# huj31415/nbody3d-webgpu

Hardware: AMD Instinct MI355X
Metric: pair-interactions/s (higher is better)
Workload: dtype f32; 1 GPU; N=262144 Plummer sphere, dt=1e-3, G=1, eps2=1e-4, i-sharded over 1 GPU(s); n=262144, kernel_variant=f32pk_symw_ipl16_j1_w2048_r32t128, parallelism=1gpu

## Files before the change

include/nbody3d_hip.h:

```cpp
#ifndef NBODY3D_HIP_H
#define NBODY3D_HIP_H

#include <stddef.h>
#include <stdint.h>

#ifdef __cplusplus
extern "C" {
#endif
#if defined(__GNUC__)
#pragma GCC visibility push(default)
#endif

#define NB_ABI_VERSION 2u
#define NB_ABI_MINOR 4u

typedef struct nb_sim nb_sim;

typedef enum nb_status {
    NB_OK = 0,
    NB_ERR_INVALID = 1,
    NB_ERR_NO_DEVICE = 2,
    NB_ERR_HIP = 3,
    NB_ERR_STATE = 4,
    NB_ERR_NOMEM = 5,
    NB_ERR_COMM = 6,
    NB_NOT_READY = 7
} nb_status;

typedef enum nb_precision { NB_F32 = 0, NB_F64 = 1 } nb_precision;

#define NB_FLAG_EXT_STREAM 1u
#define NB_FLAG_LDS_ONLY 4u
#define NB_FLAG_NO_FUSE 8u
#define NB_FLAG_POISON 16u

#define NB_FLAG_JPK_FENCED 32u

#define NB_FLAG_NO_SYM 64u

#define NB_FLAG_SYM_SHARD 128u

#define NB_FLAG_WHOLE_SWEEPS 256u

#define NB_FLAG_SINGLE_SWEEPS 512u

typedef enum nb_array { NB_BODIES = 0, NB_VEL = 1, NB_ACCEL = 2, NB_JERK = 3  } nb_array;

typedef enum nb_integrator { NB_INT_LEAPFROG = 0, NB_INT_HERMITE4 = 1 } nb_integrator;

typedef struct nb_config {
    uint32_t struct_size;
    uint32_t n;
    uint32_t precision;
    uint32_t tile;
    double eps2;
    int32_t device;
    uint32_t shard_begin;
    uint32_t shard_count;
    void *ext_stream;
    void *ext_bodies;
    uint32_t force_variant;
    uint32_t jsplit;
    uint32_t flags;
    uint32_t layer_budget_mib;
    uint32_t integrator;
    uint32_t reserved[3];
} nb_config;

uint32_t nb_abi_version(void);
uint32_t nb_abi_minor(void);

int nb_device_count(void);

int nb_create(const nb_config *cfg, nb_sim **out);

void nb_destroy(nb_sim *s);

// ... 128 lines not shown
```

nbody3d-webgpu_amd/csrc/kernels/symmetric.hip.h:

```cpp
#pragma once

namespace nb {

template <typename T> struct SymRowT { T x, y, z; };
using SymRow = SymRowT<float>;

constexpr uint32_t kFlushSteps = 4096;

template <int NG>
__device__ __forceinline__ void flush_resident_sums(float (*hi)[64], const int lane, const bool flushed, nb_f2 (&ax)[NG], nb_f2 (&ay)[NG], nb_f2 (&az)[NG])
{
    if (flushed) {
#pragma unroll
        for (int c = 0; c < NG; ++c) {
            hi[6 * c + 0][lane] += ax[c].x; hi[6 * c + 1][lane] += ay[c].x; hi[6 * c + 2][lane] += az[c].x;
            hi[6 * c + 3][lane] += ax[c].y; hi[6 * c + 4][lane] += ay[c].y; hi[6 * c + 5][lane] += az[c].y;
        }
    } else {
#pragma unroll
        for (int c = 0; c < NG; ++c) {
            hi[6 * c + 0][lane] = ax[c].x; hi[6 * c + 1][lane] = ay[c].x; hi[6 * c + 2][lane] = az[c].x;
            hi[6 * c + 3][lane] = ax[c].y; hi[6 * c + 4][lane] = ay[c].y; hi[6 * c + 5][lane] = az[c].y;
        }
    }
// ... 147 lines not shown
#pragma unroll
    for (int c = 0; c < NG; ++c) {
        out[(2 * c) * 64] = SymRow{ax[c].x, ay[c].x, az[c].x};
        out[(2 * c + 1) * 64] = SymRow{ax[c].y, ay[c].y, az[c].y};
    }
}

struct SymWK { uint32_t np, nsb, W, total_hi, total_lo, n_hi, zc, ups, r_layer0, t_layer0; };
#define SYMW_PLAN_PARAMS const uint32_t W_, const uint32_t ups_, const uint32_t nsb_, const uint32_t zc_, const uint32_t r_layer0_, const uint32_t t_layer0_
typedef uint32_t nb_u4 __attribute__((ext_vector_type(4)));
template <int TAIL>
__device__ __forceinline__ void symw_record_and_tail(const uint32_t* rec_at, nb_u4& rec, uint32_t (&tail)[TAIL])
{
    static_assert(TAIL == 1 || TAIL == 4, "f32: eps2; f64: G, eps2");
    constexpr int kTailOffset = 4 * 8 + 6 * 4;
    if constexpr (TAIL == 1) {
        asm volatile("s_load_dwordx4 %0, %2, 0x0\n\ts_load_dword %1, %3, %4\n\ts_waitcnt lgkmcnt(0)"
                     : "=&s"(rec), "=&s"(tail[0]) : "s"(rec_at), "s"(__builtin_amdgcn_kernarg_segment_ptr()), "n"(kTailOffset) : "memory");
    } else {
        nb_u4 t;
        asm volatile("s_load_dwordx4 %0, %2, 0x0\n\ts_load_dwordx4 %1, %3, %4\n\ts_waitcnt lgkmcnt(0)"
                     : "=&s"(rec), "=&s"(t) : "s"(rec_at), "s"(__builtin_amdgcn_kernarg_segment_ptr()), "n"(kTailOffset) : "memory");
        tail[0] = t.x; tail[1] = t.y; tail[2] = t.z; tail[3] = t.w;
    }
}

__device__ __forceinline__ SymWK symw_plan_words(uint32_t S, uint32_t cps, uint32_t W, uint32_t ups, uint32_t nsb, uint32_t zc, uint32_t r_layer0, uint32_t t_layer0)
{
    const uint32_t H = (nsb - 1u) >> 1, n_hi = (nsb & 1u) ? 0u : nsb >> 1;
    const uint32_t total_lo = (H + 1u) * cps + zc, total_hi = total_lo + (n_hi ? cps : 0u);
    return SymWK{(nsb + (zc ? 1u : 0u)) * S, nsb, W, total_hi, total_lo, n_hi, zc, ups, r_layer0, t_layer0};
}

template <int NG, int J, bool PAIR>
__device__ __forceinline__ void symw_sweeps(const uint32_t* __restrict__ gtab, const float4* __restrict__ bodies, SymRow* __restrict__ partial, SymRow* __restrict__ spill,
                                            SYMW_PLAN_PARAMS, uint32_t* __restrict__ queue, const uint32_t npieces, const uint32_t pieces_off)
{
    static_assert(!PAIR || J == 1, "paired sweeps: one traveler per lane and sweep");
    constexpr uint32_t S = 128u * NG;
    constexpr int GW = NG < 4 ? NG : 4;
    constexpr uint32_t CH = 64u * J;
    constexpr uint32_t CPS = S / CH;
    const SymWK pl = symw_plan_words(S, CPS, W_, ups_, nsb_, zc_, r_layer0_, t_layer0_);
    const int lane = threadIdx.x & 63, wi = threadIdx.x >> 6;
    const uint32_t w = __builtin_amdgcn_readfirstlane(blockIdx.x * 4u + wi);
    const bool active = w < pl.W;
    NB_STAMP(0);
    __shared__ float red[4][6 * NG][64];
    __shared__ uint32_t fin[4];
    const uint32_t ups = pl.ups, ush = (uint32_t)__builtin_ctz(ups), ustep = 64u >> ush,
                   tab1 = 2u * (pl.np / S);
    nb_u4 rec;
    uint32_t tail[1];
    symw_record_and_tail(gtab + tab1 + 4u * (active ? w : 0u), rec, tail);
    const float eps2 = __builtin_bit_cast(float, tail[0]);
    const nb_f2 e2 = nb_f2{eps2, eps2};
    const uint32_t first_lo = pl.n_hi * pl.total_hi, first_z = first_lo + (pl.nsb - pl.n_hi) * pl.total_lo;
    const uint32_t slot = rec.w;
    NB_STAMP_LIGHT(1);
    bool first_part = true;

    auto run = [&](uint32_t u, const uint32_t uend, const uint32_t piece_layer) -> uint32_t {
        uint32_t gfin = ~0u;
        while (u < uend) {
            const uint32_t p = u >> ush;
            uint32_t g, k, total;
            if (p < first_lo) { g = p / pl.total_hi; k = p - g * pl.total_hi; total = pl.total_hi; }
            else if (p < first_z) { const uint32_t r = p - first_lo; g = pl.n_hi + r / pl.total_lo; k = r - (g - pl.n_hi) * pl.total_lo; total = pl.total_lo; }
            else { g = pl.nsb; k = p - first_z; total = pl.zc; }
            const uint32_t ring = g < pl.nsb ? total - CPS - pl.zc : 0u;
            const uint32_t both_end = g < pl.nsb ? ring + pl.zc : 0u;
            uint32_t ug_end = (p - k + total) * ups;
            if (ug_end > uend) ug_end = uend;

            nb_f2 xi[NG], yi[NG], zi[NG], mi[NG], ax[NG], ay[NG], az[NG];
            {
                const float4* rb = bodies + (size_t)g * S + lane;
#pragma unroll
                for (int c = 0; c < NG; ++c) {
                    const float4 b0 = ld4(rb + (2 * c) * 64), b1 = ld4(rb + (2 * c + 1) * 64);
                    xi[c] = nb_f2{b0.x, b1.x}; yi[c] = nb_f2{b0.y, b1.y}; zi[c] = nb_f2{b0.z, b1.z}; mi[c] = nb_f2{b0.w, b1.w};
                    ax[c] = nb_f2{0, 0}; ay[c] = nb_f2{0, 0}; az[c] = nb_f2{0, 0};
                }
            }
            uint32_t since = 0;
            bool flushed = false;
            while (u < ug_end) {
                const uint32_t q0 = u & (ups - 1u);
                bool pair = false;
                if constexpr (PAIR) pair = q0 == 0u && ug_end - u >= 2u * ups && k + 1u < both_end;
                uint32_t nun = ups - q0;
                if (nun > ug_end - u) nun = ug_end - u;
                const uint32_t s0 = q0 * ustep, s1 = s0 + nun * ustep;
                u += pair ? 2u * ups : nun;
                if (since >= kFlushSteps) {
                    flush_resident_sums<NG>(red[wi], lane, flushed, ax, ay, az);
                    flushed = true;
                    since = 0;
                }
                since += pair ? 128u : s1 - s0;
                const bool sym = k < both_end, zsweep = k >= ring && sym;
                const uint32_t d = k / CPS;
                uint32_t tb = g + 1 + d;
                if (tb >= pl.nsb) tb -= pl.nsb;
                const uint32_t tstart = k < ring ? tb * S + (k % CPS) * CH : zsweep ? pl.nsb * S + (k - ring) * CH : g * S + (k - both_end) * CH;
                const uint32_t zrow = g * pl.zc + (k - ring);
                ++k;
                if constexpr (PAIR) {
                    if (pair) {
                        const bool zsweep1 = k >= ring;
                        const uint32_t d1 = k / CPS;
                        uint32_t tb1 = g + 1 + d1;
                        if (tb1 >= pl.nsb) tb1 -= pl.nsb;
                        const uint32_t tstart1 = zsweep1 ? pl.nsb * S + (k - ring) * CH : tb1 * S + (k % CPS) * CH;
                        const uint32_t zrow1 = g * pl.zc + (k - ring);
                        ++k;
                        const float4 t0 = ld4(bodies + tstart + lane), t1 = ld4(bodies + tstart1 + lane);
                        nb_f2 tx = nb_f2{t0.x, t1.x}, ty = nb_f2{t0.y, t1.y}, tz = nb_f2{t0.z, t1.z}, tm = nb_f2{t0.w, t1.w};
                        float bx0 = 0, bx1 = 0, by0 = 0, by1 = 0, bz0 = 0, bz1 = 0;
                        if (first_part) NB_STAMP(2);
                        for (uint32_t st = 0; st < 64u; ++st) {
                            nb_f2 sx = nb_f2{0, 0}, sy = nb_f2{0, 0}, sz = nb_f2{0, 0};
#pragma unroll
                            for (int c0g = 0; c0g < NG; c0g += GW) {
#pragma unroll
                                for (int f = 0; f < 2; ++f) {
                                    nb_f2 dx[GW], dy[GW], dz[GW], d2[GW], r[GW], si[GW], sj[GW];
#pragma unroll
                                    for (int c = 0; c < GW; ++c) dx[c] = symw_sub(f, tx, xi[c0g + c]);
#pragma unroll
                                    for (int c = 0; c < GW; ++c) dy[c] = symw_sub(f, ty, yi[c0g + c]);
#pragma unroll
                                    for (int c = 0; c < GW; ++c) dz[c] = symw_sub(f, tz, zi[c0g + c]);
#pragma unroll
                                    for (int c = 0; c < GW; ++c) d2[c] = __builtin_elementwise_fma(dx[c], dx[c], e2);
#pragma unroll
                                    for (int c = 0; c < GW; ++c) d2[c] = __builtin_elementwise_fma(dy[c], dy[c], d2[c]);
#pragma unroll
                                    for (int c = 0; c < GW; ++c) d2[c] = __builtin_elementwise_fma(dz[c], dz[c], d2[c]);
#pragma unroll
                                    for (int c = 0; c < GW; ++c) r[c] = d2[c] * d2[c];
#pragma unroll
                                    for (int c = 0; c < GW; ++c) r[c] = r[c] * d2[c];
#pragma unroll
                                    for (int c = 0; c < GW; ++c) r[c] = nb_f2{nb_rsq(r[c].x), nb_rsq(r[c].y)};
#pragma unroll
                                    for (int c = 0; c < GW; ++c) si[c] = symw_mul(f, tm, r[c]);
#pragma unroll
                                    for (int c = 0; c < GW; ++c) sj[c] = mi[c0g + c] * r[c];
#pragma unroll
                                    for (int c = 0; c < GW; ++c) ax[c0g + c] = __builtin_elementwise_fma(si[c], dx[c], ax[c0g + c]);
#pragma unroll
                                    for (int c = 0; c < GW; ++c) ay[c0g + c] = __builtin_elementwise_fma(si[c], dy[c], ay[c0g + c]);
#pragma unroll
                                    for (int c = 0; c < GW; ++c) az[c0g + c] = __builtin_elementwise_fma(si[c], dz[c], az[c0g + c]);
#pragma unroll
                                    for (int c = 0; c < GW; ++c) sx = symw_fnma(f, sj[c], dx[c], sx);
#pragma unroll
                                    for (int c = 0; c < GW; ++c) sy = symw_fnma(f, sj[c], dy[c], sy);
#pragma unroll
                                    for (int c = 0; c < GW; ++c) sz = symw_fnma(f, sj[c], dz[c], sz);
                                }
                            }
                            tx = nb_f2{wave_rot1(tx.x), wave_rot1(tx.y)}; ty = nb_f2{wave_rot1(ty.x), wave_rot1(ty.y)};
                            tz = nb_f2{wave_rot1(tz.x), wave_rot1(tz.y)}; tm = nb_f2{wave_rot1(tm.x), wave_rot1(tm.y)};
                            wave_rot1_add(bx0, sx.x); wave_rot1_add(bx1, sx.y); wave_rot1_add(by0, sy.x); wave_rot1_add(by1, sy.y);
                            wave_rot1_add(bz0, sz.x); wave_rot1_add(bz1, sz.y);
                            __builtin_amdgcn_sched_barrier(0);
                        }
                        if (first_part) { NB_STAMP_LIGHT(3); first_part = false; }
                        const uint32_t home = ((uint32_t)lane + 1u) & 63u;
                        SymRow* out0 = (zsweep ? spill + (size_t)zrow * CH : partial + (size_t)(pl.t_layer0 + d) * pl.np + tstart) + home;
                        SymRow* out1 = (zsweep1 ? spill + (size_t)zrow1 * CH : partial + (size_t)(pl.t_layer0 + d1) * pl.np + tstart1) + home;
                        *out0 = SymRow{bx0, by0, bz0};
                        *out1 = SymRow{bx1, by1, bz1};
                        continue;
                    }
                }
                float tx[J], ty[J], tz[J], tm[J];
                nb_f2 bx[J], by[J], bz[J];
                const uint32_t src = ((uint32_t)lane - s0) & 63u;
#pragma unroll
                for (int uu = 0; uu < J; ++uu) {
                    const float4 t = ld4(bodies + tstart + uu * 64 + src);
                    tx[uu] = t.x; ty[uu] = t.y; tz[uu] = t.z; tm[uu] = t.w;
                    bx[uu] = nb_f2{0, 0}; by[uu] = nb_f2{0, 0}; bz[uu] = nb_f2{0, 0};
                }
                auto steps = [&](auto both) {
                    constexpr bool BOTH = decltype(both)::value;
                    for (uint32_t st = s0; st < s1; ++st) {
#pragma unroll
                        for (int uu = 0; uu < J; ++uu) {
                            const nb_f2 px = nb_f2{tx[uu], tx[uu]}, py = nb_f2{ty[uu], ty[uu]}, pz = nb_f2{tz[uu], tz[uu]}, pm = nb_f2{tm[uu], tm[uu]};
#pragma unroll
                            for (int c0g = 0; c0g < NG; c0g += GW) {
                                nb_f2 dx[GW], dy[GW], dz[GW], d2[GW], r[GW], si[GW], sj[GW];
#pragma unroll
                                for (int c = 0; c < GW; ++c) dx[c] = px - xi[c0g + c];
#pragma unroll
                                for (int c = 0; c < GW; ++c) dy[c] = py - yi[c0g + c];
#pragma unroll
// ... 105 lines not shown
            members += same;
            mine += same && j < wi;
        }
        SymRow* out = partial + (size_t)(pl.r_layer0 + rec.z) * pl.np + (size_t)gfin * S + lane;
        for (int r = mine; r < 2 * NG; r += members) {
            float sx = 0.f, sy = 0.f, sz = 0.f;
#pragma unroll
            for (int j = 0; j < 4; ++j)
                if (fin[j] == gfin) { sx += red[j][3 * r + 0][lane]; sy += red[j][3 * r + 1][lane]; sz += red[j][3 * r + 2][lane]; }
            out[r * 64] = SymRow{sx, sy, sz};
        }
    }
    if (npieces) {
        for (;;) {
            uint32_t id = 0;
            if (lane == 0) id = __hip_atomic_fetch_add(queue, 1u, __ATOMIC_RELAXED, __HIP_MEMORY_SCOPE_AGENT);
            id = __builtin_amdgcn_readfirstlane(id);
            if (id >= npieces) break;
            const uint32_t pu = gtab[pieces_off + 2u * id], ll = gtab[pieces_off + 2u * id + 1u];
            (void)run(pu, pu + (ll >> 16), ll & 0xffffu);
        }
    }
    NB_STAMP(4);
}

#define SYMW_KERNEL_PARAMS const uint32_t* __restrict__ gtab, const float4* __restrict__ bodies, SymRow* __restrict__ partial, SymRow* __restrict__ spill, \
                           SYMW_PLAN_PARAMS, const float eps2_arg ,                       \
                           uint32_t* __restrict__ queue, const uint32_t npieces, const uint32_t pieces_off
#define SYMW_KERNEL_ARGS gtab, bodies, partial, spill, W_, ups_, nsb_, zc_, r_layer0_, t_layer0_, queue, npieces, pieces_off
template <int NG, int J>
__global__ __launch_bounds__(256) __attribute__((amdgpu_waves_per_eu(NG >= 4 ? 2 : 4, NG > 4 ? 2 : (NG < 4 ? 8 : 4))))
void nb_force_symw(SYMW_KERNEL_PARAMS)
{
    symw_sweeps<NG, J, false>(SYMW_KERNEL_ARGS);
}
template <int NG>
__global__ __launch_bounds__(256) __attribute__((amdgpu_waves_per_eu(2, NG > 4 ? 2 : 4)))
void nb_force_symw_pairs(SYMW_KERNEL_PARAMS)
{
    symw_sweeps<NG, 1, true>(SYMW_KERNEL_ARGS);
}

__device__ __forceinline__ double wave_rot1(double v)
{
    const long long b = __builtin_bit_cast(long long, v);
    const int lo = (int)(b & 0xffffffffll), hi = (int)(b >> 32);
    const unsigned rlo = (unsigned)__builtin_amdgcn_update_dpp(lo, lo, 0x13C, 0xF, 0xF, false);
    const unsigned rhi = (unsigned)__builtin_amdgcn_update_dpp(hi, hi, 0x13C, 0xF, 0xF, false);
    return __builtin_bit_cast(double, (long long)(((unsigned long long)rhi << 32) | rlo));
}

template <int IPL>
__global__ __launch_bounds__(256) __attribute__((amdgpu_waves_per_eu(2, 2)))
void nb_force_symw64(const uint32_t* __restrict__ gtab, const double4* __restrict__ bodies, SymRowT<double>* __restrict__ partial, SymRowT<double>* __restrict__ spill,
                     SYMW_PLAN_PARAMS, const double G_arg, const double eps2_arg ,
                     uint32_t* __restrict__ queue, const uint32_t npieces, const uint32_t pieces_off)
{
    constexpr uint32_t S = 64u * IPL, CH = 64u, CPS = S / CH;
    const SymWK pl = symw_plan_words(S, CPS, W_, ups_, nsb_, zc_, r_layer0_, t_layer0_);
    constexpr int GW = 4;
    const int lane = threadIdx.x & 63, wi = threadIdx.x >> 6;
    const uint32_t w = __builtin_amdgcn_readfirstlane(blockIdx.x * 4u + wi);
    const bool active = w < pl.W;
    __shared__ double red[4][3 * IPL][64];
    __shared__ uint32_t fin[4];
    const uint32_t ups = pl.ups, ush = (uint32_t)__builtin_ctz(ups), ustep = 64u >> ush,
                   tab1 = 2u * (pl.np / S);
    nb_u4 rec;
    uint32_t tail[4];
    symw_record_and_tail(gtab + tab1 + 4u * (active ? w : 0u), rec, tail);
    const double G = __builtin_bit_cast(double, (unsigned long long)tail[1] << 32 | tail[0]), eps2 = __builtin_bit_cast(double, (unsigned long long)tail[3] << 32 | tail[2]);
    const uint32_t first_lo = pl.n_hi * pl.total_hi, first_z = first_lo + (pl.nsb - pl.n_hi) * pl.total_lo;
    const uint32_t slot = rec.w;
// ... 586 lines not shown
```

nbody3d-webgpu_amd/csrc/nb_engine.hip:

```cpp
#include "nb_internal.h"
#include "nb_kernels.hip.h"
#include "../../include/nbody3d_hip_plan.h"

#include <hip/hip_ext.h>

#include <algorithm>
#include <cmath>
#include <cstdio>
#include <cstdlib>
#include <cstring>
#include <new>
#include <type_traits>

namespace {
thread_local std::string g_create_error = "";
}

namespace nbi {
int fail(nb_sim* s, int code, const std::string& msg)
{
    if (s) s->err = msg; else g_create_error = msg;
    return code;
}
void set_create_error(const std::string& msg) { g_create_error = msg; }
// ... 60 lines not shown
NB_PK_TABLE(pk_fused_kernel, nb_step_fused)

template <typename T>
const void* scalar_kernel(int ipl, int ls)
{
    if (ls == 1) {
        if (ipl == 1) return (const void*)&nb::nb_force<T, 1, 1>;
        if (ipl == 2) return (const void*)&nb::nb_force<T, 2, 1>;
        if (ipl == 4) return (const void*)&nb::nb_force<T, 4, 1>;
        return nullptr;
    }
    if (ipl != 1) return nullptr;
    if (ls == 4) return (const void*)&nb::nb_force<T, 1, 4>;
    if (ls == 16) return (const void*)&nb::nb_force<T, 1, 16>;
    if (ls == 64) return (const void*)&nb::nb_force<T, 1, 64>;
    return nullptr;
}

const void* sgpr_kernel(int ipl, int ws)
{
    if (ipl == 4 && ws == 5) return (const void*)&nb::nb_force_pk_sgpr<2, 4, true>;
    if (ipl == 4) return ws == 4 ? (const void*)&nb::nb_force_pk_sgpr<2, 4> : (const void*)&nb::nb_force_pk_sgpr<2, 1>;
    if (ipl == 8 && ws == 5) return (const void*)&nb::nb_force_pk_sgpr<4, 4, true>;
    if (ipl == 8) return ws == 4 ? (const void*)&nb::nb_force_pk_sgpr<4, 4> : (const void*)&nb::nb_force_pk_sgpr<4, 1>;
    return nullptr;
}

const void* rank_kernel_of(bool f64, int ipl)
{
    if (f64) return ipl == 8 ? (const void*)&nb::nb_force_symw64_rank<8> : nullptr;
    return ipl == 16 ? (const void*)&nb::nb_force_symw_rank<8> : ipl == 8 ? (const void*)&nb::nb_force_symw_rank<4> : nullptr;
}

const void* kernel_of(bool f64, const Shape& sh, bool single_sweeps = false)
{
    switch (sh.kind) {
        case kScalar: return f64 ? scalar_kernel<double>(sh.ipl, sh.ls) : scalar_kernel<float>(sh.ipl, sh.ls);
        case kPkLds: return f64 || (sh.ipl & 1) ? nullptr : pk_force_kernel(sh.ipl / 2, sh.ls, sh.x);
        case kFused: return f64 || (sh.ipl & 1) ? nullptr : pk_fused_kernel(sh.ipl / 2, sh.ls, sh.x);
        case kPkSgpr: return f64 || sh.ls != 1 || !(sh.x == 1 || sh.x == 4 || sh.x == 5) ? nullptr : sgpr_kernel(sh.ipl, sh.x);
        case kDirect:
            if (f64 || sh.ipl != 2 || sh.ls != 64) return nullptr;
            return sh.x == 1 ? (const void*)&nb::nb_step_direct<16> : sh.x == 2 ? (const void*)&nb::nb_step_direct<32> : nullptr;
        case kSym:
            if (sh.ls != 1) return nullptr;
            if (f64) return sh.ipl == 8 && sh.x == 3 ? (const void*)&nb::nb_force_symw64<8> : nullptr;
            if (sh.x == 4) return sh.ipl == 8 ? (const void*)&nb::nb_force_sym<4, 4, 2> : nullptr;
            if (sh.ipl == 4) return sh.x == 3 ? (const void*)&nb::nb_force_symw<2, 1> : nullptr;
            if (sh.ipl == 8 && sh.x == 3) return single_sweeps ? (const void*)&nb::nb_force_symw<4, 1> : (const void*)&nb::nb_force_symw_pairs<4>;
            if (sh.ipl == 16 && sh.x == 3) return single_sweeps ? (const void*)&nb::nb_force_symw<8, 1> : (const void*)&nb::nb_force_symw_pairs<8>;
            if (sh.ipl == 8) return sh.x == 1 ? (const void*)&nb::nb_force_symw<4, 2> : nullptr;
            if (sh.ipl == 16) return sh.x == 1 ? (const void*)&nb::nb_force_symw<8, 2> : nullptr;
            return nullptr;
        case kJpk:
            if (f64 || sh.ipl != 1 || sh.ls != 1) return nullptr;
            return sh.x == 4 ? (const void*)&nb::nb_step_jpk<4> : sh.x == 8 ? (const void*)&nb::nb_step_jpk<8>
                   : sh.x == 6 ? (const void*)&nb::nb_step_jpk<16> : nullptr;
        default: return nullptr;
    }
}

void plan_handle(nb_sim* s, const nb_config& cfg, int n_cu, double clock_hz, double device_mem)
{
    PlanInput in;
    if (device_mem > 0) in.device_mem = device_mem;
    in.n = s->n; in.sb = s->sb; in.sc = s->sc; in.f64 = s->f64; in.cfg = cfg; in.n_cu = n_cu; in.clock_hz = clock_hz;
    if (!s->no_device)
        in.occupancy = [f64 = s->f64](const Shape& sh, int block) {
            int occ = 0;
            const void* fn = kernel_of(f64, sh);
            if (!fn || hipOccupancyMaxActiveBlocksPerMultiprocessor(&occ, fn, block, 0) != hipSuccess) { (void)hipGetLastError(); return 0; }
            return occ;
        };
    LaunchPlan p = plan_launch(in);
    s->ipl = p.ipl; s->ls = p.ls; s->ws = p.ws; s->tl = p.tl;
    s->packed = p.packed; s->sgpr = p.sgpr; s->fused = p.fused; s->direct = p.direct; s->jpk = p.jpk; s->swap_acc = p.swap_acc;
    s->jsplit = p.jsplit; s->j_per_split = p.j_per_split; s->junits = p.junits; s->own_split0 = p.own_split0; s->own_splits = p.own_splits;
    s->sym = p.sym; s->symw = p.symw; s->sym_rank = p.sym_rank;
    s->sym_np = p.sym_np; s->sym_layers = p.sym_layers; s->sym_g0 = p.sym_g0; s->sym_g1 = p.sym_g1;
    static_assert(sizeof(s->sym_plan) == sizeof(p.sym_plan), "nb_sim::sym_plan mirrors LaunchPlan::sym_plan");
    memcpy(s->sym_plan, p.sym_plan, sizeof s->sym_plan);
    static_assert(sizeof(s->sym_rank_plan) == sizeof(p.sym_rank_plan), "nb_sim::sym_rank_plan mirrors LaunchPlan::sym_rank_plan");
    memcpy(s->sym_rank_plan, p.sym_rank_plan, sizeof s->sym_rank_plan);
// ... 62 lines not shown
        const void* b = jstream(s, s->cur);
        void* p = s->partial;
        const uint32_t* tab = s->sym_tab + ps.tab_off;
        uint32_t n = s->n, k_lo = ps.k_lo, k_hi = ps.k_hi, d0 = ps.d0;
        void* sp = s->sym_spill;
        if (s->f64) {
            double G = s->G, e2 = s->eps2;
            void* args[] = {&b, &p, &tab, &rp, &n, &G, &e2, &w0, &w1, &sp, &k_lo, &k_hi, &d0};
            launch_kernel(rank_kernel_of(true, sh.ipl), dim3(ceil_div(w1 - w0, 4u)), dim3(256), args, s->stream, t0, t1);
        } else {
            float e2 = (float)s->eps2;
            void* args[] = {&b, &p, &tab, &rp, &n, &e2, &w0, &w1, &sp, &k_lo, &k_hi, &d0};
            launch_kernel(rank_kernel_of(false, sh.ipl), dim3(ceil_div(w1 - w0, 4u)), dim3(256), args, s->stream, t0, t1);
        }
        return;
    }
    if (s->symw) {
        nb::SymWPlan pl;
        memcpy(&pl, s->sym_plan, sizeof pl);
        const void* b = jstream(s, s->cur);
        void* p = s->partial;
        const uint32_t* tab = s->sym_tab;
        void* sp = s->sym_spill;
        uint32_t* queue = s->sym_queue;
        uint32_t npieces = s->sym_pieces, pieces_off = 2u * (pl.np / ipb_of(sh)) + 4u * pl.W;
        if (npieces) (void)hipMemsetAsync(queue, 0, sizeof(uint32_t), s->stream);
        if (s->f64) {
            double G = s->G, e2 = s->eps2;
            void* args[] = {&tab, &b, &p, &sp, &pl.W, &pl.ups, &pl.nsb, &pl.zc, &pl.r_layer0, &pl.t_layer0, &G, &e2, &queue, &npieces, &pieces_off};
            launch_kernel(kernel_of(true, sh), dim3(ceil_div(pl.W, 4u)), dim3(256), args, s->stream, t0, t1);
        } else {
            float e2 = (float)s->eps2;
            void* args[] = {&tab, &b, &p, &sp, &pl.W, &pl.ups, &pl.nsb, &pl.zc, &pl.r_layer0, &pl.t_layer0, &e2, &queue, &npieces, &pieces_off};
            launch_kernel(kernel_of(false, sh, s->single_sweeps), dim3(ceil_div(pl.W, 4u)), dim3(256), args, s->stream, t0, t1);
        }
        return;
    }
    if (s->sym) {
        nb::SymPlan pl;
        memcpy(&pl, s->sym_plan, sizeof pl);
        const float4* b = (const float4*)jstream(s, s->cur);
        nb::SymRow* p = (nb::SymRow*)s->partial;
        float e2 = (float)s->eps2;
        uint32_t n = s->n;
        void* args[] = {&b, &p, &pl, &n, &e2};
        launch_kernel(kernel_of(false, sh), dim3(pl.nsb * pl.q), dim3(64 * sh.x), args, s->stream, t0, t1);
        return;
    }
    nb::SplitWindow win{0, 0xffffffffu, 0};
    uint32_t ny = s->jsplit;
    if (part == 1) { win.base = s->own_split0; ny = s->own_splits; }
    else if (part == 2) { win.hole_begin = s->own_split0; win.hole_count = s->own_splits; ny = s->jsplit - s->own_splits; }
    if (ny == 0) return;
    dim3 grid(ceil_div(s->sc, ipb_of(sh)), ny), block(nb::kBlock);
    const V4* b = (const V4*)jstream(s, s->cur);
    V4* p = (V4*)s->partial;
    T G = (T)s->G, e2 = (T)s->eps2;
    uint32_t n = s->n, sb = s->sb, sc = s->sc, jps = s->j_per_split;
    const V4* zr = (const V4*)s->zero_row;
    void* args[] = {&b, &p, &n, &sb, &sc, &G, &e2, &jps, &win, &zr};
    launch_kernel(kernel_of(s->f64, sh), grid, block, args, s->stream, t0, t1);
}

void ensure_pairs(nb_sim* s)
{
    if (!s->jpk || (s->pairs_ok && s->pairs_G == s->G)) return;
    const float4* b = (const float4*)s->bodies[s->cur];
// ... 520 lines not shown
        s->hermite = true;
        fj_shape(s->n, s->f64, n_cu, &s->fj_chunks, &s->fj_per);
        s->jsplit = s->fj_chunks; s->j_per_split = s->fj_per;
        s->variant = std::string("hermite4_") + (s->f64 ? "f64" : "f32pk") + "_c" + std::to_string(s->fj_chunks) + "_j" + std::to_string(s->fj_per);
        const size_t hrow = 4 * s->esz;
        NB_HIPC(hipMalloc(&s->bodies[0], hrow * s->n));
        s->own_bodies = true;
        for (void** p : {&s->vel, &s->acc, &s->jerk, &s->hx, &s->hv}) NB_HIPC(hipMalloc(p, hrow * s->n));
        NB_HIPC(hipMalloc(&s->fj_part, (size_t)2 * hrow * s->fj_chunks * s->n));
        NB_HIPC(hipMalloc(&s->zero_row, 64));
        NB_HIPC(hipMemsetAsync(s->zero_row, 0, 64, s->stream));
        s->diag_chunk = nb::kTile * std::min(16u, std::max(1u, s->n / 16384u));
        s->diag_blocks = ceil_div(s->sc, nb::kDiagRows) * ceil_div(s->n, s->diag_chunk);
        NB_HIPC(hipMalloc((void**)&s->diag, sizeof(double) * 5 * s->diag_blocks));
        *out = s;
        return NB_OK;
    }
    plan_handle(s, cfg, n_cu, clock_hz, (double)prop.totalGlobalMem);
    if (s->sym && (!s->sym_rank || s->sym_local) && !cfg.force_variant) {
        size_t free_b = 0, total_b = 0;
        auto need = [&]() { return 3.0 * s->esz * (double)sym_layer_rows(s) * s->sym_layers + 12.0 * s->esz * s->sym_np; };
        if (hipMemGetInfo(&free_b, &total_b) == hipSuccess && need() > 0.9 * (double)free_b) {
            nb_config fit = cfg;
            fit.layer_budget_mib = (uint32_t)std::max(1.0, 0.6 * (double)free_b / 1048576.0);
            plan_handle(s, fit, n_cu, clock_hz, (double)prop.totalGlobalMem);
            if (s->sym && need() > 0.9 * (double)free_b) {
                cfg.flags |= NB_FLAG_NO_SYM;
                plan_handle(s, cfg, n_cu, clock_hz, (double)prop.totalGlobalMem);
            }
        }
    }
    if (!kernel_of(s->f64, shape_of(s))) return bail(NB_ERR_INVALID, "nb_create: no kernel for shape " + s->variant);
    s->single_sweeps = (cfg.flags & NB_FLAG_SINGLE_SWEEPS) != 0;

    const size_t row = 4 * s->esz;
    if (cfg.ext_bodies) { s->bodies[0] = cfg.ext_bodies; s->own_bodies = false; }
    else {
        const size_t rows = s->sym ? s->sym_np : s->n;
        NB_HIPC(hipMalloc(&s->bodies[0], row * rows));
        if (s->sym) NB_HIPC(hipMemset(s->bodies[0], 0, row * rows));
        s->own_bodies = true;
        if (s->fused) NB_HIPC(hipMalloc(&s->bodies[1], row * s->n));
    }
    NB_HIPC(hipMalloc(&s->vel, row * s->sc));
    NB_HIPC(hipMalloc(&s->acc, row * s->sc));
    auto alloc_partial = [&](size_t bytes) -> hipError_t {
        if (s->partial) return hipErrorInvalidValue;
        s->partial_bytes = bytes;
        return hipMalloc(&s->partial, bytes);
    };
    if (s->sym) {
        NB_HIPC(alloc_partial((size_t)3 * s->esz * sym_layer_rows(s) * s->sym_layers));
        if (s->sym_rank) NB_HIPC(hipMalloc(&s->sym_A, 4 * s->esz * s->sym_np));
        if (s->sym_spill_rows) {
            NB_HIPC(hipMalloc(&s->sym_spill, (size_t)3 * s->esz * s->sym_spill_rows));
            NB_HIPC(hipMemset(s->sym_spill, 0, (size_t)3 * s->esz * s->sym_spill_rows));
        }
        if (s->symw && s->sym_pieces) {
            NB_HIPC(hipMalloc((void**)&s->sym_queue, 64));
            NB_HIPC(hipMemset(s->sym_queue, 0, 64));
        }
        if (s->symw) {
            NB_HIPC(hipMalloc((void**)&s->sym_tab, sizeof(uint32_t) * s->sym_tab_host.size()));
            NB_HIPC(hipMemcpy(s->sym_tab, s->sym_tab_host.data(), sizeof(uint32_t) * s->sym_tab_host.size(), hipMemcpyHostToDevice));
        }
    } else if (!s->fused) {
// ... 834 lines not shown
```

nbody3d-webgpu_amd/csrc/nb_internal.h:

```cpp
#pragma once
#include "../../include/nbody3d_hip.h"
#include "nb_plan.h"

#include <hip/hip_runtime.h>

#include <cstdint>
#include <string>
#include <vector>

struct nb_events { hipEvent_t e[8]; bool two, xchg, rs, blk; };

struct nb_rccl;

struct nb_frame_slot {
    float* h_bodies = nullptr;
    float* h_speed = nullptr;
    float* d_bodies = nullptr;
    float* d_speed = nullptr;
    hipEvent_t packed = nullptr;
    hipEvent_t landed = nullptr;
    uint64_t step = 0;
    bool in_flight = false, valid = false;
};

// ... 21 lines not shown
    uint32_t diag_blocks = 0, diag_chunk = 256;
    double dt = 0.0, G = 0.0;
    bool params_set = false, uploaded = false;
    uint64_t steps_done = 0;
    int ipl = 1, ls = 1;
    bool packed = false;
    bool sgpr = false;
    int ws = 1;
    int tl = 1;
    bool fused = false;
    bool direct = false;
    bool jpk = false;
    void* pairs[2] = {nullptr, nullptr};
    bool pairs_ok = false;
    double pairs_G = 0.0;
    void* jpartial = nullptr;
    uint32_t* tickets = nullptr;
    uint32_t junits = 0;
    bool poison = false;
    bool jpk_fenced = false;
    int acc_parity = 0;
    bool swap_acc = false;
    uint32_t jsplit = 1, j_per_split = 0;
    bool sym = false;
    uint32_t sym_np = 0, sym_layers = 0;
    uint32_t sym_plan[16] = {0};
    bool symw = false;
    uint32_t* sym_tab = nullptr;
    std::vector<uint32_t> sym_tab_host;
    void* sym_spill = nullptr;
    uint32_t sym_spill_rows = 0;
    uint32_t sym_pieces = 0;
    bool single_sweeps = false;
    uint32_t* sym_queue = nullptr;
    bool sym_rank = false;
    uint32_t sym_g0 = 0, sym_g1 = 0;
    uint32_t sym_rank_plan[16] = {0};
    std::vector<nbp::LaunchPlan::SymPass> sym_passes;
    uint32_t sym_pass = 0;
    bool sym_local = false;
    void* sym_A = nullptr;
    std::string variant, err;
    nb_exchange_fn xfn = nullptr;
    nb_exchange_wait_fn xwait = nullptr;
    void* xuser = nullptr;
    bool gather_pending = false;
    uint32_t own_split0 = 0, own_splits = 0;
    nb_rccl* rccl = nullptr;
    bool timing = false;
    struct graph_slot {
        hipGraph_t graph = nullptr;
        hipGraphExec_t exec = nullptr;
        double dt = 0.0, G = 0.0;
        int parity = 0;
    } graphs[2];
    bool graphs_ok = true;
    std::vector<nb_events> pool;
    std::vector<nb_events> pending;
    size_t pool_next = 0;
    hipStream_t frame_stream = nullptr;
    static constexpr int kFrameSlots = 4;
    nb_frame_slot frame[kFrameSlots];
    int frame_next = 0;
    int frame_latest = -1;
    int n_cu = 256;
    struct field_buf { void* p = nullptr; size_t cap = 0; } fld_pts, fld_acc, fld_phi, fld_part;
// ... 38 lines not shown
```

nbody3d-webgpu_amd/nbody3d_amd/capi.py:

```python
import ctypes as C
import os

import numpy as np

_PKG = os.path.dirname(os.path.abspath(__file__))
_LIB_PATH = os.environ.get("NB_ENGINE_LIB") or os.path.normpath(os.path.join(_PKG, "..", "csrc", "libnbody3d_hip.so"))

NB_F32, NB_F64 = 0, 1
NB_FLAG_EXT_STREAM = 1
NB_FLAG_LDS_ONLY = 4
NB_FLAG_NO_FUSE = 8
NB_FLAG_POISON = 16
NB_FLAG_JPK_FENCED = 32
NB_FLAG_NO_SYM = 64
NB_FLAG_SYM_SHARD = 128
NB_FLAG_WHOLE_SWEEPS = 256
NB_FLAG_SINGLE_SWEEPS = 512
NB_RCCL_ID_BYTES = 128
NB_RCCL_OVERLAP = 1
NB_MULTI_PEER, NB_MULTI_RCCL, NB_MULTI_PEER_OVERLAP = 0, 1, 2
NB_NOT_READY = 7
NB_FIELD_AT_BODIES, NB_FIELD_F64, NB_FIELD_DEVICE = 1, 2, 4
NB_INT_LEAPFROG, NB_INT_HERMITE4 = 0, 1
INTEGRATORS = {"leapfrog": NB_INT_LEAPFROG, "hermite4": NB_INT_HERMITE4}
STATUS = {0: "NB_OK", 1: "NB_ERR_INVALID", 2: "NB_ERR_NO_DEVICE", 3: "NB_ERR_HIP",
          4: "NB_ERR_STATE", 5: "NB_ERR_NOMEM", 6: "NB_ERR_COMM", 7: "NB_NOT_READY"}
ABI_VERSION = 2
ABI_MINOR = 3


class NBodyError(RuntimeError):
    def __init__(self, code, msg):
        super().__init__("%s: %s" % (STATUS.get(code, code), msg))
        self.code = code


class nb_config(C.Structure):
    _fields_ = [
        ("struct_size", C.c_uint32), ("n", C.c_uint32), ("precision", C.c_uint32), ("tile", C.c_uint32),
        ("eps2", C.c_double), ("device", C.c_int32), ("shard_begin", C.c_uint32), ("shard_count", C.c_uint32),
        ("ext_stream", C.c_void_p), ("ext_bodies", C.c_void_p),
        ("force_variant", C.c_uint32), ("jsplit", C.c_uint32), ("flags", C.c_uint32), ("layer_budget_mib", C.c_uint32),
        ("integrator", C.c_uint32), ("reserved", C.c_uint32 * 3),
    ]


class nb_plan_info(C.Structure):
    _fields_ = [("struct_size", C.c_uint32)] + [(k, C.c_uint32) for k in (
        "kind", "ipl", "ls", "x", "jsplit", "j_per_split", "own_split0", "own_splits",
        "sym", "symw", "sym_rank", "sym_np", "sym_layers", "sym_g0", "sym_g1")] + [
# ... 681 lines not shown
```

Baseline: 6811 billion pair-interactions/s.

## Rotate paired travelers through an LDS ring instead of DPP lane rotations

Result: no change. 6837 billion pair-interactions/s, median of 6 (+0.4%).

```diff
diff --git a/include/nbody3d_hip.h b/include/nbody3d_hip.h
--- a/include/nbody3d_hip.h
+++ b/include/nbody3d_hip.h
@@ -43,6 +43,8 @@
 #define NB_FLAG_WHOLE_SWEEPS 256u
 
 #define NB_FLAG_SINGLE_SWEEPS 512u
+
+#define NB_FLAG_DPP_PAIRS 1024u
 
 typedef enum nb_array { NB_BODIES = 0, NB_VEL = 1, NB_ACCEL = 2, NB_JERK = 3  } nb_array;
 
diff --git a/nbody3d-webgpu_amd/csrc/kernels/symmetric.hip.h b/nbody3d-webgpu_amd/csrc/kernels/symmetric.hip.h
--- a/nbody3d-webgpu_amd/csrc/kernels/symmetric.hip.h
+++ b/nbody3d-webgpu_amd/csrc/kernels/symmetric.hip.h
@@ -203,11 +203,77 @@
     return SymWK{(nsb + (zc ? 1u : 0u)) * S, nsb, W, total_hi, total_lo, n_hi, zc, ups, r_layer0, t_layer0};
 }
 
-template <int NG, int J, bool PAIR>
+enum SymwPairs { kNoPairs, kDppPairs, kLdsPairs };
+
+typedef float nb_f4 __attribute__((ext_vector_type(4)));
+template <int OFF>
+__device__ __forceinline__ void symw_ring_read(nb_f4& e0, nb_f4& e1, const uint32_t at)
+{
+    asm volatile("ds_read_b128 %0, %2 offset:%3\n\tds_read_b128 %1, %2 offset:%4" : "=&v"(e0), "=&v"(e1) : "v"(at), "n"(OFF), "n"(OFF + 2048) : "memory");
+}
+__device__ __forceinline__ void symw_ring_wait() { asm volatile("s_waitcnt lgkmcnt(0)" : : : "memory"); }
+template <int OFF>
+__device__ __forceinline__ void symw_ring_wait_step_read(uint32_t& at, nb_f4& n0, nb_f4& n1)
+{
+    asm volatile("s_waitcnt lgkmcnt(0)\n\tv_subrev_u32_e32 %0, 32, %0\n\tds_read_b128 %1, %0 offset:%3\n\tds_read_b128 %2, %0 offset:%4"
+                 : "+v"(at), "=&v"(n0), "=&v"(n1) : "n"(OFF), "n"(OFF + 2048) : "memory");
+}
+
+template <int NG>
+__device__ __forceinline__ void symw_pair_step(const nb_f2 tx, const nb_f2 ty, const nb_f2 tz, const nb_f2 tm, const nb_f2 e2,
+                                               const nb_f2 (&xi)[NG], const nb_f2 (&yi)[NG], const nb_f2 (&zi)[NG], const nb_f2 (&mi)[NG],
+                                               nb_f2 (&ax)[NG], nb_f2 (&ay)[NG], nb_f2 (&az)[NG], nb_f2& sx, nb_f2& sy, nb_f2& sz)
+{
+    constexpr int GW = NG < 4 ? NG : 4;
+    sx = nb_f2{0, 0}; sy = nb_f2{0, 0}; sz = nb_f2{0, 0};
+#pragma unroll
+    for (int c0g = 0; c0g < NG; c0g += GW) {
+#pragma unroll
+        for (int f = 0; f < 2; ++f) {
+            nb_f2 dx[GW], dy[GW], dz[GW], d2[GW], r[GW], si[GW], sj[GW];
+#pragma unroll
+            for (int c = 0; c < GW; ++c) dx[c] = symw_sub(f, tx, xi[c0g + c]);
+#pragma unroll
+            for (int c = 0; c < GW; ++c) dy[c] = symw_sub(f, ty, yi[c0g + c]);
+#pragma unroll
+            for (int c = 0; c < GW; ++c) dz[c] = symw_sub(f, tz, zi[c0g + c]);
+#pragma unroll
+            for (int c = 0; c < GW; ++c) d2[c] = __builtin_elementwise_fma(dx[c], dx[c], e2);
+#pragma unroll
+            for (int c = 0; c < GW; ++c) d2[c] = __builtin_elementwise_fma(dy[c], dy[c], d2[c]);
+#pragma unroll
+            for (int c = 0; c < GW; ++c) d2[c] = __builtin_elementwise_fma(dz[c], dz[c], d2[c]);
+#pragma unroll
+            for (int c = 0; c < GW; ++c) r[c] = d2[c] * d2[c];
+#pragma unroll
+            for (int c = 0; c < GW; ++c) r[c] = r[c] * d2[c];
+#pragma unroll
+            for (int c = 0; c < GW; ++c) r[c] = nb_f2{nb_rsq(r[c].x), nb_rsq(r[c].y)};
+#pragma unroll
+            for (int c = 0; c < GW; ++c) si[c] = symw_mul(f, tm, r[c]);
+#pragma unroll
+            for (int c = 0; c < GW; ++c) sj[c] = mi[c0g + c] * r[c];
+#pragma unroll
+            for (int c = 0; c < GW; ++c) ax[c0g + c] = __builtin_elementwise_fma(si[c], dx[c], ax[c0g + c]);
+#pragma unroll
+            for (int c = 0; c < GW; ++c) ay[c0g + c] = __builtin_elementwise_fma(si[c], dy[c], ay[c0g + c]);
+#pragma unroll
+            for (int c = 0; c < GW; ++c) az[c0g + c] = __builtin_elementwise_fma(si[c], dz[c], az[c0g + c]);
+#pragma unroll
+            for (int c = 0; c < GW; ++c) sx = symw_fnma(f, sj[c], dx[c], sx);
+#pragma unroll
+            for (int c = 0; c < GW; ++c) sy = symw_fnma(f, sj[c], dy[c], sy);
+#pragma unroll
+            for (int c = 0; c < GW; ++c) sz = symw_fnma(f, sj[c], dz[c], sz);
+        }
+    }
+}
+
+template <int NG, int J, SymwPairs PAIRS>
 __device__ __forceinline__ void symw_sweeps(const uint32_t* __restrict__ gtab, const float4* __restrict__ bodies, SymRow* __restrict__ partial, SymRow* __restrict__ spill,
                                             SYMW_PLAN_PARAMS, uint32_t* __restrict__ queue, const uint32_t npieces, const uint32_t pieces_off)
 {
-    static_assert(!PAIR || J == 1, "paired sweeps: one traveler per lane and sweep");
+    static_assert(PAIRS == kNoPairs || J == 1, "paired sweeps: one traveler per lane and sweep");
     constexpr uint32_t S = 128u * NG;
     constexpr int GW = NG < 4 ? NG : 4;
     constexpr uint32_t CH = 64u * J;
@@ -219,6 +285,12 @@
     NB_STAMP(0);
     __shared__ float red[4][6 * NG][64];
     __shared__ uint32_t fin[4];
+    uint32_t ring_at = 0;
+    if constexpr (PAIRS == kLdsPairs) {
+        __shared__ nb_f4 ring[4][2][128];
+        static_assert(sizeof(ring) + sizeof(red) + sizeof(fin) <= 81920, "two workgroups per CU");
+        ring_at = (uint32_t)(uintptr_t)(__attribute__((address_space(3))) nb_f4*)&ring[wi][0][64 + lane] - 32u;
+    }
     const uint32_t ups = pl.ups, ush = (uint32_t)__builtin_ctz(ups), ustep = 64u >> ush,
                    tab1 = 2u * (pl.np / S);
     nb_u4 rec;
@@ -259,7 +331,7 @@
             while (u < ug_end) {
                 const uint32_t q0 = u & (ups - 1u);
                 bool pair = false;
-                if constexpr (PAIR) pair = q0 == 0u && ug_end - u >= 2u * ups && k + 1u < both_end;
+                if constexpr (PAIRS != kNoPairs) pair = q0 == 0u && ug_end - u >= 2u * ups && k + 1u < both_end;
                 uint32_t nun = ups - q0;
                 if (nun > ug_end - u) nun = ug_end - u;
                 const uint32_t s0 = q0 * ustep, s1 = s0 + nun * ustep;
@@ -277,7 +349,7 @@
                 const uint32_t tstart = k < ring ? tb * S + (k % CPS) * CH : zsweep ? pl.nsb * S + (k - ring) * CH : g * S + (k - both_end) * CH;
                 const uint32_t zrow = g * pl.zc + (k - ring);
                 ++k;
-                if constexpr (PAIR) {
+                if constexpr (PAIRS != kNoPairs) {
                     if (pair) {
                         const bool zsweep1 = k >= ring;
                         const uint32_t d1 = k / CPS;
@@ -287,8 +359,34 @@
                         const uint32_t zrow1 = g * pl.zc + (k - ring);
                         ++k;
                         const float4 t0 = ld4(bodies + tstart + lane), t1 = ld4(bodies + tstart1 + lane);
+                        float bx0 = 0, bx1 = 0, by0 = 0, by1 = 0, bz0 = 0, bz1 = 0;
+                        if constexpr (PAIRS == kLdsPairs) {
+                            nb_f4 a0 = nb_f4{t0.x, t1.x, t0.y, t1.y}, a1 = nb_f4{t0.z, t1.z, t0.w, t1.w}, b0, b1;
+                            {
+                                __attribute__((address_space(3))) nb_f4* slot0 = (__attribute__((address_space(3))) nb_f4*)(uintptr_t)(ring_at + 32u);
+                                slot0[-64] = a0; slot0[0] = a0; slot0[64] = a1; slot0[128] = a1;
+                            }
+                            uint32_t at = ring_at;
+                            if (first_part) NB_STAMP(2);
+                            for (uint32_t st = 0; st < 32u; ++st) {
+                                nb_f2 sx, sy, sz;
+                                symw_ring_read<16>(b0, b1, at);
+                                __builtin_amdgcn_sched_barrier(0);
+                                symw_pair_step<NG>(nb_f2{a0.x, a0.y}, nb_f2{a0.z, a0.w}, nb_f2{a1.x, a1.y}, nb_f2{a1.z, a1.w}, e2, xi, yi, zi, mi, ax, ay, az, sx, sy, sz);
+                                wave_rot1_add(bx0, sx.x); wave_rot1_add(bx1, sx.y); wave_rot1_add(by0, sy.x); wave_rot1_add(by1, sy.y);
+                                wave_rot1_add(bz0, sz.x); wave_rot1_add(bz1, sz.y);
+                                __builtin_amdgcn_sched_barrier(0);
+                                symw_ring_wait_step_read<32>(at, a0, a1);
+                                __builtin_amdgcn_sched_barrier(0);
+                                symw_pair_step<NG>(nb_f2{b0.x, b0.y}, nb_f2{b0.z, b0.w}, nb_f2{b1.x, b1.y}, nb_f2{b1.z, b1.w}, e2, xi, yi, zi, mi, ax, ay, az, sx, sy, sz);
+                                wave_rot1_add(bx0, sx.x); wave_rot1_add(bx1, sx.y); wave_rot1_add(by0, sy.x); wave_rot1_add(by1, sy.y);
+                                wave_rot1_add(bz0, sz.x); wave_rot1_add(bz1, sz.y);
+                                __builtin_amdgcn_sched_barrier(0);
+                                symw_ring_wait();
+                                __builtin_amdgcn_sched_barrier(0);
+                            }
+                        } else {
                         nb_f2 tx = nb_f2{t0.x, t1.x}, ty = nb_f2{t0.y, t1.y}, tz = nb_f2{t0.z, t1.z}, tm = nb_f2{t0.w, t1.w};
-                        float bx0 = 0, bx1 = 0, by0 = 0, by1 = 0, bz0 = 0, bz1 = 0;
                         if (first_part) NB_STAMP(2);
                         for (uint32_t st = 0; st < 64u; ++st) {
                             nb_f2 sx = nb_f2{0, 0}, sy = nb_f2{0, 0}, sz = nb_f2{0, 0};
@@ -338,6 +436,7 @@
                             wave_rot1_add(bx0, sx.x); wave_rot1_add(bx1, sx.y); wave_rot1_add(by0, sy.x); wave_rot1_add(by1, sy.y);
                             wave_rot1_add(bz0, sz.x); wave_rot1_add(bz1, sz.y);
                             __builtin_amdgcn_sched_barrier(0);
+                        }
                         }
                         if (first_part) { NB_STAMP_LIGHT(3); first_part = false; }
                         const uint32_t home = ((uint32_t)lane + 1u) & 63u;
@@ -509,13 +608,20 @@
 __global__ __launch_bounds__(256) __attribute__((amdgpu_waves_per_eu(NG >= 4 ? 2 : 4, NG > 4 ? 2 : (NG < 4 ? 8 : 4))))
 void nb_force_symw(SYMW_KERNEL_PARAMS)
 {
-    symw_sweeps<NG, J, false>(SYMW_KERNEL_ARGS);
+    symw_sweeps<NG, J, kNoPairs>(SYMW_KERNEL_ARGS);
 }
 template <int NG>
 __global__ __launch_bounds__(256) __attribute__((amdgpu_waves_per_eu(2, NG > 4 ? 2 : 4)))
 void nb_force_symw_pairs(SYMW_KERNEL_PARAMS)
 {
-    symw_sweeps<NG, 1, true>(SYMW_KERNEL_ARGS);
+    symw_sweeps<NG, 1, kDppPairs>(SYMW_KERNEL_ARGS);
+}
+template <int NG>
+__global__ __launch_bounds__(256) __attribute__((amdgpu_waves_per_eu(2, 2)))
+void nb_force_symw_lds(SYMW_KERNEL_PARAMS)
+{
+    static_assert(NG == 8, "two workgroups per CU");
+    symw_sweeps<NG, 1, kLdsPairs>(SYMW_KERNEL_ARGS);
 }
 
 __device__ __forceinline__ double wave_rot1(double v)
diff --git a/nbody3d-webgpu_amd/csrc/nb_engine.hip b/nbody3d-webgpu_amd/csrc/nb_engine.hip
--- a/nbody3d-webgpu_amd/csrc/nb_engine.hip
+++ b/nbody3d-webgpu_amd/csrc/nb_engine.hip
@@ -116,7 +116,7 @@
     return ipl == 16 ? (const void*)&nb::nb_force_symw_rank<8> : ipl == 8 ? (const void*)&nb::nb_force_symw_rank<4> : nullptr;
 }
 
-const void* kernel_of(bool f64, const Shape& sh, bool single_sweeps = false)
+const void* kernel_of(bool f64, const Shape& sh, bool single_sweeps = false, bool dpp_pairs = false)
 {
     switch (sh.kind) {
         case kScalar: return f64 ? scalar_kernel<double>(sh.ipl, sh.ls) : scalar_kernel<float>(sh.ipl, sh.ls);
@@ -132,7 +132,8 @@
             if (sh.x == 4) return sh.ipl == 8 ? (const void*)&nb::nb_force_sym<4, 4, 2> : nullptr;
             if (sh.ipl == 4) return sh.x == 3 ? (const void*)&nb::nb_force_symw<2, 1> : nullptr;
             if (sh.ipl == 8 && sh.x == 3) return single_sweeps ? (const void*)&nb::nb_force_symw<4, 1> : (const void*)&nb::nb_force_symw_pairs<4>;
-            if (sh.ipl == 16 && sh.x == 3) return single_sweeps ? (const void*)&nb::nb_force_symw<8, 1> : (const void*)&nb::nb_force_symw_pairs<8>;
+            if (sh.ipl == 16 && sh.x == 3)
+                return single_sweeps ? (const void*)&nb::nb_force_symw<8, 1> : dpp_pairs ? (const void*)&nb::nb_force_symw_pairs<8> : (const void*)&nb::nb_force_symw_lds<8>;
             if (sh.ipl == 8) return sh.x == 1 ? (const void*)&nb::nb_force_symw<4, 2> : nullptr;
             if (sh.ipl == 16) return sh.x == 1 ? (const void*)&nb::nb_force_symw<8, 2> : nullptr;
             return nullptr;
@@ -261,7 +262,7 @@
         } else {
             float e2 = (float)s->eps2;
             void* args[] = {&tab, &b, &p, &sp, &pl.W, &pl.ups, &pl.nsb, &pl.zc, &pl.r_layer0, &pl.t_layer0, &e2, &queue, &npieces, &pieces_off};
-            launch_kernel(kernel_of(false, sh, s->single_sweeps), dim3(ceil_div(pl.W, 4u)), dim3(256), args, s->stream, t0, t1);
+            launch_kernel(kernel_of(false, sh, s->single_sweeps, s->dpp_pairs), dim3(ceil_div(pl.W, 4u)), dim3(256), args, s->stream, t0, t1);
         }
         return;
     }
@@ -848,6 +849,7 @@
     }
     if (!kernel_of(s->f64, shape_of(s))) return bail(NB_ERR_INVALID, "nb_create: no kernel for shape " + s->variant);
     s->single_sweeps = (cfg.flags & NB_FLAG_SINGLE_SWEEPS) != 0;
+    s->dpp_pairs = (cfg.flags & NB_FLAG_DPP_PAIRS) != 0;
 
     const size_t row = 4 * s->esz;
     if (cfg.ext_bodies) { s->bodies[0] = cfg.ext_bodies; s->own_bodies = false; }
diff --git a/nbody3d-webgpu_amd/csrc/nb_internal.h b/nbody3d-webgpu_amd/csrc/nb_internal.h
--- a/nbody3d-webgpu_amd/csrc/nb_internal.h
+++ b/nbody3d-webgpu_amd/csrc/nb_internal.h
@@ -77,6 +77,7 @@
     uint32_t sym_spill_rows = 0;
     uint32_t sym_pieces = 0;
     bool single_sweeps = false;
+    bool dpp_pairs = false;
     uint32_t* sym_queue = nullptr;
     bool sym_rank = false;
     uint32_t sym_g0 = 0, sym_g1 = 0;
diff --git a/nbody3d-webgpu_amd/nbody3d_amd/capi.py b/nbody3d-webgpu_amd/nbody3d_amd/capi.py
--- a/nbody3d-webgpu_amd/nbody3d_amd/capi.py
+++ b/nbody3d-webgpu_amd/nbody3d_amd/capi.py
@@ -16,6 +16,7 @@
 NB_FLAG_SYM_SHARD = 128
 NB_FLAG_WHOLE_SWEEPS = 256
 NB_FLAG_SINGLE_SWEEPS = 512
+NB_FLAG_DPP_PAIRS = 1024
 NB_RCCL_ID_BYTES = 128
 NB_RCCL_OVERLAP = 1
 NB_MULTI_PEER, NB_MULTI_RCCL, NB_MULTI_PEER_OVERLAP = 0, 1, 2
```
